# nanoporetech/pomfret

Hardware: AMD Instinct MI355X
Metric: aligned reads/sec (methphase kernel) (higher is better)
Workload: dtype u32/f32

## Files before the change

include/pomfret_amd.h:

```cpp
#ifndef POMFRET_AMD_H
#define POMFRET_AMD_H

#include <stddef.h>
#include <stdint.h>

#ifdef __cplusplus
extern "C" {
#endif

#define PF_ABI_VERSION 1

#define PF_OK               0
#define PF_ERR_ARG         -1
#define PF_ERR_HIP         -2
#define PF_ERR_NOMEM       -3
#define PF_ERR_UNSUPPORTED -4
#define PF_ERR_LIMIT       -5
#define PF_ERR_INTERNAL    -6

typedef struct pf_cfg {
    int32_t k;
    int32_t k_span;
    int32_t cov_for_selection;
    int32_t cov_for_runtime;
// ... 75 lines not shown
#define PF_VAR_D 3

typedef struct pf_known_vars {
    uint32_t n;
    const uint32_t *pos;
    const uint32_t *len;
    const uint8_t  *op;
    const uint8_t  *haptag;
    const uint64_t *char_off;
    const uint8_t  *chars;
} pf_known_vars_t;

typedef struct pf_read_aln_batch {
    uint32_t n_reads;
    const uint32_t *start;
    const uint32_t *end;
    const uint64_t *cigar_off;
    const uint32_t *cigar;
    const uint64_t *seq_off;
    const uint32_t *seq_len;
    const uint8_t  *seq;
    const uint64_t *md_off;
    const char     *md;
} pf_read_aln_batch_t;


typedef struct pf_ctx pf_ctx_t;
typedef struct pf_dbatch pf_dbatch_t;

int  pf_abi_version(void);
int  pf_device_count(void);
const char *pf_strerror(int code);

int  pf_ctx_create(int device, pf_ctx_t **out);
void pf_ctx_destroy(pf_ctx_t *ctx);

int  pf_batch_upload(pf_ctx_t *ctx, const pf_cfg_t *cfg,
                     const pf_window_batch_t *batch, pf_dbatch_t **out);
void pf_batch_free(pf_dbatch_t *db);
uint32_t pf_batch_n_windows(const pf_dbatch_t *db);
uint32_t pf_batch_n_reads(const pf_dbatch_t *db);
uint64_t pf_batch_n_calls(const pf_dbatch_t *db);

int  pf_methphase_run(pf_ctx_t *ctx, pf_dbatch_t *db, pf_window_out_t *out);

int  pf_methphase_launch(pf_ctx_t *ctx, pf_dbatch_t *db);
int  pf_methphase_finish(pf_ctx_t *ctx, pf_dbatch_t *db, pf_window_out_t *out);

int  pf_batch_upload_aln(pf_ctx_t *ctx, const pf_cfg_t *cfg, const pf_load_cfg_t *lcfg,
                         const pf_aln_batch_t *aln, pf_dbatch_t **out);
int  pf_batch_read_recs(const pf_dbatch_t *db, uint32_t *rec_of_read, uint32_t n);
int64_t pf_batch_debug_calls(pf_dbatch_t *db, uint64_t *call_off, uint32_t *pos, uint8_t *cat,
                             uint32_t *first, uint32_t *last, uint64_t cap);

int  pf_batch_debug_recs(pf_dbatch_t *db, uint64_t *sizes, uint16_t *flag, uint8_t *mapq, uint32_t *pos,
                         uint32_t *l_qseq, float *de, uint8_t *hp, uint64_t *cigar_off, uint32_t *cigar,
                         uint64_t *seq_off, uint8_t *seq, uint64_t *mm_off, uint8_t *mm, uint64_t *ml_off,
                         uint8_t *ml);
int  pf_batch_load_counters(pf_dbatch_t *db, uint64_t *out, int n);

int  pf_methphase_windows(int device, const pf_cfg_t *cfg,
                          const pf_window_batch_t *batch, pf_window_out_t *out);

int  pf_last_kernel_times(pf_ctx_t *ctx, const char **names, float *ms, int *n);

int  pf_batch_stats(pf_dbatch_t *db, uint64_t *out, uint64_t n);
int  pf_batch_k3_paths(pf_dbatch_t *db, uint8_t *out, uint64_t n);
int  pf_batch_k12_paths(pf_dbatch_t *db, uint8_t *out, uint64_t n);
int  pf_batch_k12_chunk_items(pf_dbatch_t *db, uint32_t *out);

int  pf_batch_set_mask(pf_dbatch_t *db, const uint32_t *pos, uint64_t n, const uint32_t *win_rng);
int  pf_batch_masked_sites(pf_dbatch_t *db, uint32_t *out, uint64_t n);
int  pf_batch_k3_budget(const pf_dbatch_t *db, uint32_t *out, uint64_t n);

int  pf_batch_heavy(const pf_dbatch_t *db, uint32_t *probs, uint32_t cap);

int  pf_batch_debug_sites(pf_dbatch_t *db, uint32_t w, int dir, uint32_t *real,
                          uint32_t *starts, uint8_t *lens, uint32_t cap);
int64_t pf_batch_debug_methmers(pf_dbatch_t *db, int dir, uint32_t *mmr_n,
                                uint32_t *mmr_start, uint32_t *keys, uint64_t cap);

typedef struct pf_pileup {
    uint32_t n_windows;
    uint64_t n_sites;
    const uint64_t *win_off;
    const uint32_t *pos;
    const uint32_t *cnt;
    float ms_kernels;
} pf_pileup_t;
int  pf_batch_pileup(pf_ctx_t *ctx, pf_dbatch_t *db, const uint8_t *read_hp, uint32_t n_hp, pf_pileup_t **out);
void pf_pileup_free(pf_pileup_t *p);

typedef struct pf_dmr_cfg {
    uint32_t min_cov;
    uint32_t min_delta_pct;
    uint32_t max_gap;
    uint32_t min_sites;
} pf_dmr_cfg_t;

#define PF_DMR_OPEN_LEFT  1u
#define PF_DMR_OPEN_RIGHT 2u
typedef struct pf_dmr_run {
    uint32_t start;
    uint32_t end;
    uint32_t n_sites;
    int32_t  sign;
// ... 609 lines not shown
```

pomfret_amd/_lib.py:

```python
from __future__ import annotations

import ctypes as C
import os
import weakref

import numpy as np

from .abi import (DMR_HMM_SITES, DMR_RUN_DTYPE, REGION_SUM_DTYPE, PfRegions, HmmConfig, PfDmrHmm, PfDmrHmmCfg, AlnBatch, AssignConfig, PfAssign, PfAssignCfg, Config, DmrConfig, KnownVars, LoadConfig, PfAlnBatch, PfCfg, PfDmr, PfDmrCfg,
                  PfKnownVars, PfLoadCfg, PfPerm, PfPileup, PfReadAlnBatch, PfTagcheck, PfWindowBatch, PfWindowOut, ReadAlnBatch,
                  WindowBatch, WindowResult)

_HERE = os.path.dirname(os.path.abspath(__file__))
LIB_PATH = os.path.join(_HERE, "libpomfret_amd.so")
_lib = None


class PomfretError(RuntimeError):
    pass


def lib():
    global _lib
    if _lib is None:
        if not os.path.exists(LIB_PATH):
            raise PomfretError(f"{LIB_PATH} not built: run __graft_entry__.build() or "
                               f"`make -C pomfret_amd/csrc`")
        L = C.CDLL(LIB_PATH)
        L.pf_abi_version.restype = C.c_int
        L.pf_device_count.restype = C.c_int
        L.pf_strerror.restype = C.c_char_p
        L.pf_strerror.argtypes = [C.c_int]
        L.pf_ctx_create.argtypes = [C.c_int, C.POINTER(C.c_void_p)]
        L.pf_ctx_destroy.argtypes = [C.c_void_p]
        L.pf_selftest.argtypes = [C.c_void_p, C.POINTER(C.c_uint64)]
        L.pf_batch_upload.argtypes = [C.c_void_p, C.POINTER(PfCfg), C.POINTER(PfWindowBatch),
                                      C.POINTER(C.c_void_p)]
        L.pf_batch_free.argtypes = [C.c_void_p]
        L.pf_batch_n_windows.argtypes = [C.c_void_p]
        L.pf_batch_n_windows.restype = C.c_uint32
        L.pf_batch_n_reads.argtypes = [C.c_void_p]
        L.pf_batch_n_reads.restype = C.c_uint32
        L.pf_batch_n_calls.argtypes = [C.c_void_p]
        L.pf_batch_n_calls.restype = C.c_uint64
        L.pf_methphase_run.argtypes = [C.c_void_p, C.c_void_p, C.POINTER(PfWindowOut)]
        L.pf_methphase_launch.argtypes = [C.c_void_p, C.c_void_p]
        L.pf_methphase_finish.argtypes = [C.c_void_p, C.c_void_p, C.POINTER(PfWindowOut)]
        L.pf_methphase_windows.argtypes = [C.c_int, C.POINTER(PfCfg), C.POINTER(PfWindowBatch),
                                           C.POINTER(PfWindowOut)]
        L.pf_last_kernel_times.argtypes = [C.c_void_p, C.POINTER(C.c_char_p),
                                           C.POINTER(C.c_float), C.POINTER(C.c_int)]
        L.pf_batch_stats.argtypes = [C.c_void_p, C.c_void_p, C.c_uint64]
        L.pf_batch_heavy.argtypes = [C.c_void_p, C.c_void_p, C.c_uint32]
        L.pf_batch_k3_paths.argtypes = [C.c_void_p, C.c_void_p, C.c_uint64]
        L.pf_batch_k12_paths.argtypes = [C.c_void_p, C.c_void_p, C.c_uint64]
        L.pf_batch_k3_budget.argtypes = [C.c_void_p, C.c_void_p, C.c_uint64]
        L.pf_batch_set_mask.argtypes = [C.c_void_p, C.c_void_p, C.c_uint64, C.c_void_p]
        L.pf_batch_masked_sites.argtypes = [C.c_void_p, C.c_void_p, C.c_uint64]
        L.pf_batch_debug_sites.argtypes = [C.c_void_p, C.c_uint32, C.c_int, C.c_void_p,
                                           C.c_void_p, C.c_void_p, C.c_uint32]
        L.pf_batch_debug_methmers.argtypes = [C.c_void_p, C.c_int, C.c_void_p, C.c_void_p,
                                              C.c_void_p, C.c_uint64]
        L.pf_batch_debug_methmers.restype = C.c_int64
        L.pf_fisher_exact.argtypes = [C.c_int] * 4 + [C.POINTER(C.c_double)] * 3
        L.pf_fisher_exact.restype = C.c_double
        L.pf_batch_upload_aln.argtypes = [C.c_void_p, C.POINTER(PfCfg), C.POINTER(PfLoadCfg),
                                          C.POINTER(PfAlnBatch), C.POINTER(C.c_void_p)]
        L.pf_batch_read_recs.argtypes = [C.c_void_p, C.c_void_p, C.c_uint32]
        L.pf_batch_debug_calls.argtypes = [C.c_void_p] + [C.c_void_p] * 5 + [C.c_uint64]
        L.pf_batch_debug_calls.restype = C.c_int64
        L.pf_batch_load_counters.argtypes = [C.c_void_p, C.c_void_p, C.c_int]
        L.pf_batch_debug_recs.argtypes = [C.c_void_p] * 16
        L.pf_bgzf_inflate.argtypes = [C.c_void_p, C.c_void_p, C.c_uint64, C.c_void_p, C.c_uint64,
                                      C.POINTER(C.c_uint64), C.c_void_p, C.c_uint32, C.POINTER(C.c_float)]
        L.pf_batch_pileup.argtypes = [C.c_void_p, C.c_void_p, C.c_void_p, C.c_uint32,
                                      C.POINTER(C.POINTER(PfPileup))]
        L.pf_pileup_free.argtypes = [C.POINTER(PfPileup)]
        L.pf_write_hapmeth.argtypes = [C.c_char_p, C.c_char_p, C.POINTER(PfPileup), C.c_uint32, C.c_uint32, C.c_int]
        L.pf_dmr_regions.argtypes = [C.c_void_p, C.POINTER(PfPileup), C.c_uint32, C.c_uint32, C.POINTER(PfDmrCfg),
                                     C.c_void_p, C.c_uint32, C.POINTER(C.POINTER(PfDmr))]
        L.pf_dmr_regions_block.argtypes = [C.c_void_p, C.POINTER(PfPileup), C.c_uint32, C.c_uint32, C.POINTER(PfDmrCfg),
                                           C.c_void_p, C.c_uint32, C.c_uint32, C.POINTER(C.POINTER(PfDmr))]
        L.pf_dmr_free.argtypes = [C.POINTER(PfDmr)]
        L.pf_dmr_hmm_regions.argtypes = [C.c_void_p, C.POINTER(PfPileup), C.c_uint32, C.c_uint32, C.POINTER(PfDmrCfg),
                                         C.POINTER(PfDmrHmmCfg), C.c_void_p, C.c_uint32, C.c_uint32, C.c_uint32,
                                         C.POINTER(C.POINTER(PfDmrHmm))]
        L.pf_dmr_hmm_free.argtypes = [C.POINTER(PfDmrHmm)]
        L.pf_dmr_hmm_evidence.argtypes = [C.c_uint32] * 4
        L.pf_dmr_hmm_evidence.restype = C.c_int64
        L.pf_region_sums.argtypes = [C.c_void_p, C.POINTER(PfPileup), C.c_uint32, C.c_uint32, C.POINTER(PfDmrCfg),
                                     C.c_void_p, C.c_void_p, C.c_uint64, C.c_uint32, C.POINTER(C.POINTER(PfRegions))]
        L.pf_regions_free.argtypes = [C.POINTER(PfRegions)]
        L.pf_dmr_acc_new.argtypes = [C.POINTER(PfDmrCfg), C.c_void_p, C.c_uint32]
        L.pf_dmr_acc_new.restype = C.c_void_p
        L.pf_dmr_acc_add.argtypes = [C.c_void_p, C.POINTER(PfDmr)]
        L.pf_dmr_acc_flush.argtypes = [C.c_void_p, C.POINTER(C.POINTER(PfDmr))]
        L.pf_dmr_acc_free.argtypes = [C.c_void_p]
        L.pf_write_dmr.argtypes = [C.c_char_p, C.c_char_p, C.POINTER(PfDmr), C.c_double, C.c_int]
        L.pf_batch_permtest.argtypes = [C.c_void_p, C.c_void_p, C.c_void_p, C.c_uint32, C.c_uint32, C.c_uint32,
                                        C.POINTER(C.POINTER(PfPerm))]
        L.pf_perm_free.argtypes = [C.POINTER(PfPerm)]
        L.pf_write_dmr_perm.argtypes = [C.c_char_p, C.c_char_p, C.POINTER(PfDmr), C.POINTER(PfPerm), C.c_double, C.c_int]
        L.pf_batch_assign.argtypes = [C.c_void_p, C.c_void_p, C.c_void_p, C.c_uint32, C.POINTER(PfAssignCfg),
                                      C.POINTER(C.POINTER(PfAssign))]
        L.pf_assign_free.argtypes = [C.POINTER(PfAssign)]
        L.pf_ilog2_q16.argtypes = [C.c_uint32]
        L.pf_ilog2_q16.restype = C.c_uint32
        L.pf_assign_site_weights.argtypes = [C.c_uint32] * 4 + [C.POINTER(C.c_int32)]
        L.pf_assign_site_weights.restype = None
        L.pf_write_assign.argtypes = [C.c_char_p, C.c_char_p, C.POINTER(PfAssign), C.c_void_p, C.c_void_p, C.c_void_p,
                                      C.c_void_p, C.c_char_p, C.c_int, C.POINTER(C.c_uint64)]
        L.pf_batch_tagcheck.argtypes = [C.c_void_p, C.c_void_p, C.c_void_p, C.c_uint32, C.POINTER(PfAssignCfg),
                                        C.POINTER(C.POINTER(PfTagcheck))]
        L.pf_tagcheck_free.argtypes = [C.POINTER(PfTagcheck)]
        L.pf_tagcheck_site_weights.argtypes = [C.c_uint32] * 5 + [C.POINTER(C.c_int32), C.POINTER(C.c_uint8)]
        L.pf_tagcheck_site_weights.restype = None
        L.pf_write_tagcheck.argtypes = [C.c_char_p, C.c_char_p, C.POINTER(PfTagcheck), C.c_void_p, C.c_void_p, C.c_void_p,
                                        C.c_void_p, C.c_char_p, C.c_int, C.POINTER(C.c_uint64)]
        L.pf_write_tagcheck_regions.argtypes = [C.c_char_p, C.c_char_p, C.POINTER(PfTagcheck), C.c_void_p, C.c_void_p,
                                                C.c_int, C.POINTER(C.c_uint64)]
        if hasattr(L, "pf_haptag_reads"):
            L.pf_haptag_reads.argtypes = [C.c_void_p, C.POINTER(PfKnownVars),
                                          C.POINTER(PfReadAlnBatch), C.c_void_p]
# ... 385 lines not shown

    def debug_recs(self) -> dict:
        sz = np.zeros(5, np.uint64)
        _check(lib().pf_batch_debug_recs(self.handle, sz.ctypes.data, *([None] * 14)), "pf_batch_debug_recs")
        n, nc, ns, nm, nl = (int(x) for x in sz)
        d = dict(flag=np.zeros(n, np.uint16), mapq=np.zeros(n, np.uint8), pos=np.zeros(n, np.uint32),
                 l_qseq=np.zeros(n, np.uint32), de=np.zeros(n, np.float32), hp=np.zeros(n, np.uint8),
                 cigar_off=np.zeros(n + 1, np.uint64), cigar=np.zeros(max(nc, 1), np.uint32),
                 seq_off=np.zeros(n + 1, np.uint64), seq=np.zeros(max(ns, 1), np.uint8),
                 mm_off=np.zeros(n + 1, np.uint64), mm=np.zeros(max(nm, 1), np.uint8),
                 ml_off=np.zeros(n + 1, np.uint64), ml=np.zeros(max(nl, 1), np.uint8))
        keys = ["flag", "mapq", "pos", "l_qseq", "de", "hp", "cigar_off", "cigar", "seq_off", "seq", "mm_off", "mm",
                "ml_off", "ml"]
        _check(lib().pf_batch_debug_recs(self.handle, sz.ctypes.data, *[d[k].ctypes.data for k in keys]),
               "pf_batch_debug_recs")
        d["cigar"], d["seq"], d["mm"], d["ml"] = d["cigar"][:nc], d["seq"][:ns], d["mm"][:nm], d["ml"][:nl]
        return d

    @property
    def n_reads(self) -> int:
        return int(lib().pf_batch_n_reads(self.handle))

    def read_recs(self) -> np.ndarray:
        R = self.n_reads
        out = np.zeros(max(R, 1), np.uint32)
        rc = lib().pf_batch_read_recs(self.handle, out.ctypes.data, out.size)
        if rc != 0 and self.record_level:
            self.debug_calls(cap=0, probe=True)
            R = self.n_reads
            rc = lib().pf_batch_read_recs(self.handle, out.ctypes.data, out.size)
        _check(rc, "pf_batch_read_recs")
        return out[:R]

    def debug_calls(self, cap: int = None, probe: bool = False):
        if cap is None:
            if self.record_level and not lib().pf_batch_n_calls(self.handle):
                self.debug_calls(cap=0, probe=True)
            cap = int(lib().pf_batch_n_calls(self.handle))
        R = self.n_reads
        off = np.zeros(R + 1, np.uint64)
        pos = np.zeros(max(cap, 1), np.uint32)
        cat = np.zeros(max(cap, 1), np.uint8)
        first = np.zeros(max(R, 1), np.uint32)
        last = np.zeros(max(R, 1), np.uint32)
        n = lib().pf_batch_debug_calls(self.handle, off.ctypes.data, pos.ctypes.data, cat.ctypes.data,
                                       first.ctypes.data, last.ctypes.data, cap)
        if probe:
            return None
        if n < 0:
            _check(int(n), "pf_batch_debug_calls")
        R = self.n_reads
        return off[:R + 1], pos[:n], cat[:n], first[:R], last[:R]

    def load_counters(self) -> dict:
        out = np.zeros(8, np.uint64)
        _check(lib().pf_batch_load_counters(self.handle, out.ctypes.data, 8), "pf_batch_load_counters")
        return dict(seq_path=int(out[0]), unsorted=int(out[1]), implicit=int(out[2]), bad_mm=int(out[3]),
                    dup_chunks=int(out[4]), multi_cm=int(out[5]))

    def free(self):
        if self.handle:
            lib().pf_batch_free(self.handle)
            self.handle = None

    def __del__(self):
        try:
            self.free()
        except Exception:
            pass

    def run(self, out: WindowResult = None) -> WindowResult:
        fresh = out is None
        if fresh:
            out = WindowResult.alloc(self.n_windows, self.n_reads)
        o = out.to_c()
        _check(lib().pf_methphase_run(self.ctx.handle, self.handle, C.byref(o)), "pf_methphase_run")
        if fresh:
            out.read_hp = out.read_hp[:self.n_reads]
        return out

    def pileup(self, read_hp=None) -> dict:
        hp_ptr, n_hp = None, 0
        if read_hp is not None:
            hp = np.zeros(np.size(read_hp) + 1, np.uint8)
            hp[:-1] = np.asarray(read_hp, np.uint8).ravel()
            hp_ptr, n_hp = hp.ctypes.data, hp.size - 1
        p = C.POINTER(PfPileup)()
        _check(lib().pf_batch_pileup(self.ctx.handle, self.handle, hp_ptr, n_hp, C.byref(p)), "pf_batch_pileup")
        try:
            r = p.contents
            W, n = int(r.n_windows), int(r.n_sites)
            win_off = np.ctypeslib.as_array(r.win_off, (W + 1,)).copy()
            pos = np.ctypeslib.as_array(r.pos, (n,)).copy() if n else np.zeros(0, np.uint32)
            cnt = np.ctypeslib.as_array(r.cnt, (n * 6,)).copy() if n else np.zeros(0, np.uint32)
            return dict(win_off=win_off, pos=pos, cnt=cnt.reshape(n, 3, 2), ms=float(r.ms_kernels))
        finally:
            lib().pf_pileup_free(p)

    def permtest(self, n_perm: int, seed: int = 1, read_hp=None) -> dict:
        hp_ptr, n_hp = None, 0
        if read_hp is not None:
            hp = np.zeros(np.size(read_hp) + 1, np.uint8)
            hp[:-1] = np.asarray(read_hp, np.uint8).ravel()
            hp_ptr, n_hp = hp.ctypes.data, hp.size - 1
        if not 0 <= int(n_perm) <= 0xFFFFFFFF or not 0 <= int(seed) <= 0xFFFFFFFF:
            raise PomfretError("pf_batch_permtest: n_perm and seed are 32-bit unsigned")
# ... 161 lines not shown
```

pomfret_amd/csrc/pf_api.hip:

```cpp
#include <hip/hip_runtime.h>
#include <mutex>
#include <stdint.h>
#include <stdio.h>
#include <stdlib.h>
#include <string.h>
#include <algorithm>
#include <thread>
#include <vector>
#include "pf_device.h"
#include "pf_load.h"
#include "pf_host.h"
#include "../../include/pomfret_amd.h"

__global__ void pf_k12_sites_methmers(pf_dev_batch d);
__global__ void pf_k2_methmers(pf_dev_batch d);
__global__ void pf_k12_chunks(pf_dev_batch d);
__global__ void pf_k3_greedy(pf_dev_batch d);
__global__ void pf_k3_wave(pf_dev_batch d);
__global__ void pf_k3_fallback(pf_dev_batch d);
__global__ void pf_k3_heavy(pf_dev_batch d);
__global__ void pf_k3_kdict(pf_dev_batch d);
__global__ void pf_k0_load(pf_load_dev d);
__global__ void pf_k0_multi(pf_load_dev d);
__global__ void pf_k0_scan(pf_load_dev d);
// ... 1604 lines not shown
        }
    }
    *n = tot;
    return PF_OK;
}

extern "C" int64_t pf_batch_debug_calls(pf_dbatch_t *b, uint64_t *call_off, uint32_t *pos, uint8_t *cat,
                                        uint32_t *first, uint32_t *last, uint64_t cap) {
    if (!b || !call_off || !pos || !cat || !first || !last) return PF_ERR_ARG;
    const int rc = run_debug(b, 0);
    if (rc) return rc;
    if (b->N > cap) return PF_ERR_ARG;
    if (b->R == 0) { call_off[0] = 0; return 0; }
    const uint32_t *dpos = b->d.call_pos;
    const uint8_t *dcat = b->d.call_cat;
    if (b->has_aln) {
        std::vector<uint64_t> beg(b->R), end(b->R);
        HIPCHK(hipMemcpy(beg.data(), b->d.read_call_off, 8ull * b->R, hipMemcpyDeviceToHost));
        HIPCHK(hipMemcpy(end.data(), b->d.read_call_end, 8ull * b->R, hipMemcpyDeviceToHost));
        call_off[0] = 0;
        for (uint32_t r = 0; r < b->R; r++) call_off[r + 1] = call_off[r] + (end[r] - beg[r]);
        if (call_off[b->R] != b->N) return PF_ERR_INTERNAL;
        if (b->dbg_cap < b->N || !b->dbg_off) {
            if (b->dbg_off) { free_arena(b, b->dbg_off); free_arena(b, b->dbg_pos); free_arena(b, b->dbg_cat); }
            b->dbg_off = nullptr; b->dbg_pos = nullptr; b->dbg_cat = nullptr; b->dbg_cap = 0;
            int ra = dev_alloc(b, &b->dbg_off, (size_t)b->ld.n_recs + 1);
            if (!ra) ra = dev_alloc(b, &b->dbg_pos, (size_t)b->N);
            if (!ra) ra = dev_alloc(b, &b->dbg_cat, (size_t)b->N);
            if (ra) return ra;
            b->dbg_cap = b->N;
        }
        hipStream_t st = b->ctx->stream;
        HIPCHK(hipMemcpyAsync(b->dbg_off, call_off, 8ull * (b->R + 1), hipMemcpyHostToDevice, st));
        hipLaunchKernelGGL(pf_k0_gather_calls, dim3(std::min<uint32_t>((b->R + 3) / 4, 4096)), dim3(256), 0, st,
                           b->d.read_call_off, b->dbg_off, b->R, b->d.call_pos, b->d.call_cat, b->dbg_pos, b->dbg_cat);
        HIPCHK(hipGetLastError());
        HIPCHK(hipStreamSynchronize(st));
        dpos = b->dbg_pos;
        dcat = b->dbg_cat;
    } else {
        HIPCHK(hipMemcpy(call_off, b->d.read_call_off, 8ull * (b->R + 1), hipMemcpyDeviceToHost));
    }
    if (b->N) {
        HIPCHK(hipMemcpy(pos, dpos, 4ull * b->N, hipMemcpyDeviceToHost));
        HIPCHK(hipMemcpy(cat, dcat, b->N, hipMemcpyDeviceToHost));
    }
    if (b->R) {
        HIPCHK(hipMemcpy(first, b->d.read_first, 4ull * b->R, hipMemcpyDeviceToHost));
        HIPCHK(hipMemcpy(last, b->d.read_last, 4ull * b->R, hipMemcpyDeviceToHost));
    }
    return (int64_t)b->N;
}

extern "C" int pf_batch_set_hp(pf_dbatch_t *b, const uint8_t *hp, uint32_t n) {
    if (!b || !b->has_aln || n != b->ld.n_recs || (n && !hp)) return PF_ERR_ARG;
    if (!n) return PF_OK;
    HIPCHK(hipSetDevice(b->ctx->device));
    HIPCHK(hipStreamSynchronize(b->ctx->stream));
    HIPCHK(hipMemcpy(const_cast<uint8_t *>(b->ld.hp), hp, n, hipMemcpyHostToDevice));
    return PF_OK;
}

extern "C" int pf_batch_set_mask(pf_dbatch_t *b, const uint32_t *pos, uint64_t n, const uint32_t *win_rng) {
    if (!b || (n && !pos)) return PF_ERR_ARG;
    for (uint64_t i = 0; i < n; i++) {
        if (i && pos[i] <= pos[i - 1]) return PF_ERR_ARG;
        if (pos[i] >= (1u << 29)) return PF_ERR_LIMIT;
    }
    if (n && win_rng)
        for (uint32_t w = 0; w < b->W; w++)
            if (win_rng[2 * w] > win_rng[2 * w + 1] || win_rng[2 * w + 1] > n) return PF_ERR_ARG;
    HIPCHK(hipSetDevice(b->ctx->device));
    HIPCHK(hipStreamSynchronize(b->ctx->stream));
    uint32_t *np = nullptr, *nr = nullptr;
    int rc = PF_OK;
    if (n) {
        rc = dev_put(b, &np, pos, (size_t)n);
        if (!rc && win_rng && b->W) rc = dev_put(b, &nr, win_rng, 2ull * b->W);
        if (rc) {
            if (np) free_arena(b, np);
            if (nr) free_arena(b, nr);
            return rc;
        }
    }
    pf_dev_batch &d = b->d;
    if (d.mask_pos) free_arena(b, const_cast<uint32_t *>(d.mask_pos));
    if (d.win_mask_rng) free_arena(b, const_cast<uint32_t *>(d.win_mask_rng));
    d.mask_pos = np;
    d.win_mask_rng = nr;
    d.mask_n = (uint32_t)n;
    return PF_OK;
}

extern "C" int pf_batch_masked_sites(pf_dbatch_t *b, uint32_t *out, uint64_t n) {
    if (!b || !out || n < b->W) return PF_ERR_ARG;
    HIPCHK(hipSetDevice(b->ctx->device));
    HIPCHK(hipStreamSynchronize(b->ctx->stream));
    if (b->W) HIPCHK(hipMemcpy(out, b->d.win_masked, 4ull * b->W, hipMemcpyDeviceToHost));
    return PF_OK;
}

extern "C" int pf_batch_debug_recs(pf_dbatch_t *b, uint64_t *sizes, uint16_t *flag, uint8_t *mapq, uint32_t *pos,
                                   uint32_t *l_qseq, float *de, uint8_t *hp, uint64_t *cigar_off, uint32_t *cigar,
                                   uint64_t *seq_off, uint8_t *seq, uint64_t *mm_off, uint8_t *mm, uint64_t *ml_off,
                                   uint8_t *ml) {
    if (!b || !sizes || !b->has_aln) return PF_ERR_ARG;
// ... 46 lines not shown
```

pomfret_amd/csrc/pf_load.hip:

```cpp
#include <hip/hip_runtime.h>
#include <stdint.h>
#include "pf_device.h"
#include "pf_load.h"

#define DEV static __device__ __forceinline__
#define NT_C 2u
#ifndef PF_K0_SEQ_REREAD
#define PF_K0_SEQ_REREAD 0
#endif

#ifdef PF_K0_PROFILE
DEV unsigned long long k0_now() {
    unsigned long long t;
    __builtin_amdgcn_sched_barrier(0);
    asm volatile("s_memtime %0\n\ts_waitcnt lgkmcnt(0)" : "=s"(t) :: "memory");
    __builtin_amdgcn_sched_barrier(0);
    return t;
}
#define K0_STAMP(i) do { const unsigned long long t_ = k0_now(); \
    if (d->ctr && lane == 0) atomicAdd(&d->ctr[8 + (i)], t_ - k0_t); k0_t = t_; } while (0)
#define K0_T0 unsigned long long k0_t = k0_now()
#else
#define K0_STAMP(i) do { } while (0)
#define K0_T0 do { } while (0)
#endif
#define NT_G 4u
#ifndef PF_K0_NOINL
#define PF_K0_NOINL 0
#endif
#if PF_K0_NOINL & 1
#define DEV_HBM static __device__ __attribute__((noinline))
#else
#define DEV_HBM DEV
#endif
#if PF_K0_NOINL & 2
#define DEV_COLD static __device__ __attribute__((noinline))
#else
#define DEV_COLD DEV
#endif
#ifndef PF_K0_PLACE
#define PF_K0_PLACE 1
#endif
#ifndef PF_K0_WALK2
#define PF_K0_WALK2 1
#endif
#ifndef PF_K0_FUSEC
#define PF_K0_FUSEC 1
#endif
#ifndef PF_K0_PADFIX
#define PF_K0_PADFIX 1
#endif
#ifndef PF_K0_NBRARE
#define PF_K0_NBRARE 1
#endif
#ifndef PF_K0_RANKDPP
#define PF_K0_RANKDPP 1
#endif
#ifndef PF_K0_HDRFAST
#define PF_K0_HDRFAST 1
#endif
#ifndef PF_K0_EMITDPP
#define PF_K0_EMITDPP 1
#endif
#ifndef PF_K0_DIAG1
#define PF_K0_DIAG1 0
#endif
#if PF_K0_DIAG1
#define K0_DIAG1(d) ((d)->diag == 1u)
#else
#define K0_DIAG1(d) false
#endif
#ifndef PF_K0_WPE
#define PF_K0_WPE 8
#endif

DEV uint32_t uni(uint32_t x) { return (uint32_t)__builtin_amdgcn_readfirstlane((int)x); }
DEV uint64_t lanemask_lt(uint32_t lane) { return lane ? (~0ull >> (64 - lane)) : 0ull; }
DEV uint32_t popc(uint64_t m) { return (uint32_t)__popcll(m); }
DEV uint32_t below_cnt(uint64_t b) {
    return __builtin_amdgcn_mbcnt_hi((uint32_t)(b >> 32), __builtin_amdgcn_mbcnt_lo((uint32_t)b, 0u));
}
DEV uint32_t rdl(uint32_t x, uint32_t l) { return (uint32_t)__builtin_amdgcn_readlane((int)x, (int)l); }

#define K0_CONST __attribute__((address_space(4)))
typedef const K0_CONST pf_load_dev *K0Args;
typedef const K0_CONST pf_k0_hdr *K0HdrP;
DEV K0Args k0_args() { return (K0Args)__builtin_amdgcn_kernarg_segment_ptr(); }
template <typename P>
DEV P k0_late(P p) {
    asm volatile("" : "+s"(p));
    return p;
}

DEV void wsync() {
    __builtin_amdgcn_fence(__ATOMIC_RELEASE, "workgroup");
    __builtin_amdgcn_wave_barrier();
    __builtin_amdgcn_fence(__ATOMIC_ACQUIRE, "workgroup");
}

DEV uint32_t dpp_shr_add(uint32_t x, const int ctrl) {
    uint32_t y;
    switch (ctrl) {
    case 1: y = (uint32_t)__builtin_amdgcn_update_dpp(0, (int)x, 0x111, 0xF, 0xF, true); break;
    case 2: y = (uint32_t)__builtin_amdgcn_update_dpp(0, (int)x, 0x112, 0xF, 0xF, true); break;
    case 4: y = (uint32_t)__builtin_amdgcn_update_dpp(0, (int)x, 0x114, 0xF, 0xF, true); break;
    case 8: y = (uint32_t)__builtin_amdgcn_update_dpp(0, (int)x, 0x118, 0xF, 0xF, true); break;
    case 15: y = (uint32_t)__builtin_amdgcn_update_dpp(0, (int)x, 0x142, 0xA, 0xF, false); break;
    default: y = (uint32_t)__builtin_amdgcn_update_dpp(0, (int)x, 0x143, 0xC, 0xF, false); break;
    }
    return x + y;
}
DEV uint32_t wscan(uint32_t x, uint32_t) {
    x = dpp_shr_add(x, 1);
    x = dpp_shr_add(x, 2);
    x = dpp_shr_add(x, 4);
// ... 1 lines not shown
    x = dpp_shr_add(x, 15);
    x = dpp_shr_add(x, 31);
    return x;
}
DEV uint64_t wscan64(uint64_t x, uint32_t lane) {
#pragma unroll
    for (int o = 1; o < 64; o <<= 1) {
        const uint64_t y = __shfl_up(x, o, 64);
        if (lane >= (uint32_t)o) x += y;
    }
    return x;
}
DEV uint64_t rdl64(uint64_t x, uint32_t l) {
    return ((uint64_t)rdl((uint32_t)(x >> 32), l) << 32) | rdl((uint32_t)x, l);
}

DEV uint32_t nib(const uint8_t *s, uint32_t i) { return (s[i >> 1] >> ((~i & 1u) << 2)) & 0xFu; }
DEV uint32_t nibw(uint64_t w, uint32_t i) { return (uint32_t)(w >> (8u * (i >> 1) + ((i & 1u) ? 0u : 4u))) & 0xFu; }
DEV uint32_t match16(uint64_t w, uint32_t tb, uint32_t nv) {
    uint32_t m = 0;
#pragma unroll
    for (uint32_t i = 0; i < 16; i++) m |= (nibw(w, i) == tb && i < nv) ? (1u << i) : 0u;
    return m;
}
DEV uint32_t select_bit(uint32_t m, uint32_t k) {
    for (uint32_t i = 0; i < k; i++) m &= m - 1;
    return (uint32_t)__builtin_ctz(m);
}
DEV bool is_digit(uint32_t c) { return c >= '0' && c <= '9'; }
DEV bool is_alpha(uint32_t c) { return (c >= 'a' && c <= 'z') || (c >= 'A' && c <= 'Z'); }

template <bool LE>
DEV uint32_t lb64(const uint32_t *a, uint32_t n, uint32_t v) {
    uint32_t lo = 0;
    while (n > 0) {
        const uint32_t h = n >> 1;
        const uint32_t x = a[lo + h];
        if (LE ? x <= v : x < v) { lo += h + 1; n -= h + 1; } else n = h;
    }
    return lo;
}

struct K0Merge {
    uint32_t eP[PF_K0_EC], eV[PF_K0_EC];
    uint32_t iP[PF_K0_EC], iV[PF_K0_EC];
    uint32_t mV[2 * PF_K0_EC];
    uint8_t eC[PF_K0_EC];
    uint8_t mC[2 * PF_K0_EC];
};
struct K0Seq {
    uint16_t sb[8 * 64];
    uint8_t sc[8 * 64];
};
struct K0W {
    uint32_t T[PF_K0_TCAP];
    uint32_t opE[64], opOff[64], opA[64];
    uint8_t opT[64];
    union {
        K0Seq s;
        K0Merge mg;
    } u;
};

struct K0Out {
    uint32_t n, first, last;
    uint32_t sorted, lim;
    uint32_t *pos;
    uint8_t *cat;
};

struct K0Tgt { uint32_t nd, nc, mi, th, te; uint64_t ml; };
#define PF_K0_MAXT 8
#define PF_K0_TW 7
struct K0Tgts { K0Tgt t0; uint32_t n, over; uint32_t *xt; };
DEV void k0_tgt_put(uint32_t *xt, uint32_t e, const K0Tgt &t, uint32_t lane) {
    if (lane == 0) {
        uint32_t *q = xt + PF_K0_TW * (e - 1);
        q[0] = t.nd; q[1] = t.nc; q[2] = t.mi; q[3] = t.th; q[4] = t.te; q[5] = (uint32_t)t.ml;
        q[6] = (uint32_t)(t.ml >> 32);
    }
}
DEV K0Tgt k0_tgt_get(const K0Tgts &T, uint32_t e) {
    if (e == 0) return T.t0;
    const uint32_t *q = T.xt + PF_K0_TW * (e - 1);
    K0Tgt t;
    t.nd = q[0]; t.nc = q[1]; t.mi = q[2]; t.th = q[3]; t.te = q[4];
    t.ml = ((uint64_t)q[6] << 32) | q[5];
    return t;
}

DEV uint32_t bytes_eq(uint32_t w, uint32_t c) {
    const uint32_t t = w ^ (c * 0x01010101u);
    return ~(((t & 0x7F7F7F7Fu) + 0x7F7F7F7Fu) | t) & 0x80808080u;
}
DEV uint32_t bytes_in(int32_t b, uint32_t lo, uint32_t hi) {
    const int32_t s = min(max((int32_t)lo - b, 0), 4), e = min(max((int32_t)hi - b, 0), 4);
    const uint32_t ml = s >= 4 ? 0u : 0x80808080u << (8 * s);
    const uint32_t mh = e <= 0 ? 0u : 0x80808080u >> (8 * (4 - e));
    return ml & mh;
}
DEV uint32_t wsum_small(uint32_t c) {
    return popc(__ballot(c & 1u)) + 2u * popc(__ballot(c & 2u)) + 4u * popc(__ballot(c & 4u));
}
DEV uint64_t nondigit_bytes(uint64_t y) {
    const uint64_t hi = (y & 0xF0F0F0F0F0F0F0F0ull) ^ 0x3030303030303030ull;
    const uint64_t hz = ~(((hi & 0x7F7F7F7F7F7F7F7Full) + 0x7F7F7F7F7F7F7F7Full) | hi) & 0x8080808080808080ull;
    const uint64_t ge10 = ((y & 0x0F0F0F0F0F0F0F0Full) + 0x7676767676767676ull) & 0x8080808080808080ull;
    return (~hz & 0x8080808080808080ull) | ge10;
}
DEV uint32_t swar_dec(uint64_t y, uint32_t n) {
    uint64_t z = (y & ((1ull << (8 * n)) - 1)) << (8 * (8 - n));
    z = ((z & 0x0F0F0F0F0F0F0F0Full) * 2561u) >> 8;
    z = ((z & 0x00FF00FF00FF00FFull) * 6553601u) >> 16;
    return (uint32_t)(((z & 0x0000FFFF0000FFFFull) * 42949672960001ull) >> 32);
}
// ... 338 lines not shown
DEV uint32_t u16_at(uint4 q, uint32_t e) {
    const uint32_t d = e < 2 ? q.x : e < 4 ? q.y : e < 6 ? q.z : q.w;
    return (e & 1u) ? d >> 16 : d & 0xFFFFu;
}
DEV uint64_t valid_nibbles(uint32_t nv) { return nv >= 16 ? 0x1111111111111111ull : ((1ull << (4 * nv)) - 1) & 0x1111111111111111ull; }

template <typename TP>
DEV uint32_t k0_seq_pass(K0Args d, K0W &L, const uint8_t *seq, uint32_t len, bool rev, const K0Tgt &t,
                         TP TB, uint32_t lane, bool &implicit, uint32_t &tb_off) {
    constexpr uint32_t ROWS = 8, RW = 128, BW = ROWS * RW;
    const uint64_t pat = (rev ? (uint64_t)NT_G : (uint64_t)NT_C) * 0x1111111111111111ull;
    const uint4 *sq4 = reinterpret_cast<const uint4 *>(seq);
    const uint32_t nwords = (len + 15) / 16;
    const uint32_t nblk = (nwords + BW - 1) / BW;
    const uint32_t nd = t.nd;
    auto slot = [&](uint32_t j) { return rev ? nd - 1 - j : j; };
    uint32_t carry = 0, ti = 0, nout = 0;
    bool imp = false;
    tb_off = 0;
    for (uint32_t bb = 0; bb < nblk && ti < nd; bb++) {
        const uint32_t b = rev ? nblk - 1 - bb : bb;
        uint4 v[ROWS];
        const uint32_t w0 = b * BW + 2 * lane;
        const int32_t left = (int32_t)(nwords - w0);
        const uint4 *rowp = sq4 + (w0 >> 1);
#pragma unroll
        for (uint32_t i = 0; i < ROWS; i++)
            v[i] = (int32_t)(i * RW) < left ? rowp[i * (RW / 2)] : make_uint4(0, 0, 0, 0);
        uint32_t pref[ROWS];
        uint32_t run = 0;
        auto count = [&](uint32_t i, uint32_t &c0) {
            const uint32_t w = b * BW + i * RW + 2 * lane;
            const uint64_t xs[2] = {((uint64_t)v[i].y << 32) | v[i].x, ((uint64_t)v[i].w << 32) | v[i].z};
            uint32_t c[2];
#pragma unroll
            for (uint32_t h = 0; h < 2; h++) {
#if PF_K0_PADFIX
                (void)w;
                c[h] = (uint32_t)__popcll(zero_nibbles_hi(xs[h] ^ pat));
#else
                c[h] = 0;
                if (w + h < nwords) {
                    if ((w + h) * 16 + 16 > len)
                        c[h] = (uint32_t)__popcll(zero_nibbles(nibswap(xs[h]) ^ pat) & valid_nibbles(len - (w + h) * 16));
                    else c[h] = (uint32_t)__popcll(zero_nibbles_hi(xs[h] ^ pat));
                }
#endif
            }
            c0 = c[0];
            return c[0] + c[1];
        };
#pragma unroll
        for (uint32_t i = 0; i < ROWS; i += 2) {
            uint32_t c0a, c0b;
            const uint32_t ca = count(i, c0a), cb = count(i + 1, c0b);
            L.u.s.sc[i * 64 + lane] = (uint8_t)c0a;
            L.u.s.sc[(i + 1) * 64 + lane] = (uint8_t)c0b;
            const uint32_t inc = wscan(ca | (cb << 16), lane);
            const uint32_t tot = rdl(inc, 63);
            pref[i] = run;
            const uint32_t ba = run + (inc & 0xFFFFu) - ca;
            L.u.s.sb[i * 64 + lane] = (uint16_t)ba;
            run += tot & 0xFFFFu;
            pref[i + 1] = run;
            const uint32_t bb2 = run + (inc >> 16) - cb;
            L.u.s.sb[(i + 1) * 64 + lane] = (uint16_t)bb2;
            run += tot >> 16;
#if PF_K0_PLACE
            if ((lane & 7u) == 0) {
                uint16_t *gb = reinterpret_cast<uint16_t *>(L.opA);
                gb[i * 8 + (lane >> 3)] = (uint16_t)ba;
                gb[(i + 1) * 8 + (lane >> 3)] = (uint16_t)bb2;
            }
#endif
        }
        const uint32_t btot = run;
        uint32_t tend = ti;
#if PF_K0_PLACE
        {
            const uint32_t lim = carry + btot;
            uint32_t lo = ti, n = nd - ti;
            while (n > 64) {
                const uint32_t sd = (n + 63) / 64, off = lane * sd;
                const bool in = off < n && (TB[slot(min(lo + off, nd - 1))] & 0xFFFFFFu) < lim;
                const uint32_t c = popc(__ballot(in));
                if (c == 0) { n = 0; break; }
                const uint32_t nlo = lo + (c - 1) * sd + 1;
                n = min(c * sd, n) - (c - 1) * sd - 1;
                lo = nlo;
            }
            const bool in = lane < n && (TB[slot(min(lo + lane, nd - 1))] & 0xFFFFFFu) < lim;
            tend = uni(lo + popc(__ballot(in)));
        }
#else
        {
            uint32_t n = nd - ti;
            while (n > 0) {
                const uint32_t h = n >> 1;
                if ((TB[slot(tend + h)] & 0xFFFFFFu) < carry + btot) { tend += h + 1; n -= h + 1; } else n = h;
            }
            tend = uni(tend);
        }
#endif
        wsync();
        for (uint32_t j0 = ti; j0 < (d->diag == 5u ? ti : tend); j0 += 64) {
            const uint32_t j = j0 + lane;
// ... 476 lines not shown
                const uint32_t p = key >> 2;
                const bool in = k < nT && p <= a_end;
                const uint64_t bi = __ballot(in);
                if (!bi) break;
                bool keep = false;
                uint32_t v = 0;
                if (in) {
#if PF_K0_WALK2
                    auto lt8 = [&](uint4 x, uint4 y) {
                        return (x.x < p ? 1u : 0u) + (x.y < p ? 1u : 0u) + (x.z < p ? 1u : 0u) + (x.w < p ? 1u : 0u) +
                               (y.x < p ? 1u : 0u) + (y.y < p ? 1u : 0u) + (y.z < p ? 1u : 0u) + (y.w < p ? 1u : 0u);
                    };
                    const uint4 *gl = reinterpret_cast<const uint4 *>(L.u.mg.eP);
                    const uint32_t g = lt8(gl[0], gl[1]);
                    const uint4 *ge = reinterpret_cast<const uint4 *>(L.opE + 8 * g);
                    const uint32_t oi = 8 * g + lt8(ge[0], ge[1]);
#else
                    const uint32_t oi = lb64<false>(L.opE, nv, p);
#endif
                    keep = L.opT[oi] == 0;
                    v = i_ref + p + cgoffset + L.opOff[oi];
                }
                k0_emit_lanes<MODE>(d, o, keep, v, key & 3u, false, lane, L.u.mg.mV, L.u.mg.mC);
                tc += popc(bi);
                if (popc(bi) < 64) break;
            }
        } else {
            for (uint32_t c0 = a_cur & ~3u; c0 <= a_end && (c0 < a_end || tc < nT); c0 += PF_K0_CB)
                k0_chunk_implicit<MODE>(d, L, nv, c0, a_cur, a_end, i_ref, cgoffset, rev, TB, nT, tc, seq, len,
                                        lane, o);
        }
        wsync();
        a_cur = a_end;
        off_cur = off_end;
        j += 64;
    }
    for (; j < ncig; j += 64) {
        const uint32_t g = j + lane;
        const uint32_t c = cn;
        next_tile();
        racc += k0_refc(c);
        if (trunc) continue;
        const uint32_t op = c & 15u;
        const uint64_t stop = __ballot(op == 3u || op == 4u);
        const uint64_t bad = __ballot(op > 4u && g < ncig);
        const uint32_t fs = stop ? (uint32_t)__ffsll((long long)stop) - 1 : 64u;
        const uint32_t fb = bad ? (uint32_t)__ffsll((long long)bad) - 1 : 64u;
        if (fb < fs) return false;
        trunc = fs < 64;
    }
    return true;
}

DEV K0HdrP k0_rec(K0Args d, uint32_t slot) { return (K0HdrP)(d->hdr + slot); }

template <typename TP>
DEV bool k0_merge_targets(K0Args d, K0W &L, const K0Tgts &T, uint32_t N, bool rev, TP TB,
                          const uint32_t *gw, const uint8_t *mmg, uint32_t mis, const uint8_t *ml, uint32_t mln,
                          uint32_t lane, uint32_t &nd_out, bool &past, bool &ovf) {
    nd_out = 0;
    ovf = false;
    unsigned long long t0 = 0;
    if (lane == 0) t0 = atomicAdd(d->stage_ctr, 2ull * N);
    const uint64_t cb = d->stage_off[d->n_recs] + (((uint64_t)uni((uint32_t)(t0 >> 32)) << 32) | uni((uint32_t)t0));
    if (cb + 2ull * N > d->stage_cap) {
        if (lane == 0) atomicOr(d->status, PF_ST_STAGE_OVF);
        ovf = true;
        return false;
    }
    uint32_t *tmp = d->stage_pos + cb, *mrg = tmp + N;
    k0_dw_table(L.u.mg.mV, lane);
    wsync();
    bool pst = false;
    for (uint32_t e = 0, oe = 0; e < T.n; e++) {
        const K0Tgt te = k0_tgt_get(T, e);
        uint32_t *TBe = tmp + oe;
        if (!k0_mm_ranks(gw, mmg, mis, te, rev, TBe, L.u.mg.mV, lane)) return false;
        wsync();
        for (uint32_t j = lane; j < te.nd; j += 64) {
            const uint32_t q = mln ? (uint32_t)ml[te.ml + (uint64_t)j * te.nc + te.mi] : 255u;
            const uint32_t sj = rev ? te.nd - 1 - j : j;
            const uint32_t rk = TBe[sj];
            pst |= rk >= (1u << 24);
            TBe[sj] = (rk & 0xFFFFFFu) | (q << 24);
        }
        wsync();
        oe += te.nd;
    }
    past = __ballot(pst) != 0;
    if (past) return true;
    for (uint32_t e = 0, oe = 0; e < T.n; e++) {
        const uint32_t ne = k0_tgt_get(T, e).nd;
        for (uint32_t j = lane; j < ne; j += 64) {
            const uint32_t v = tmp[oe + (rev ? ne - 1 - j : j)], rk = v & 0xFFFFFFu;
            uint32_t pos = j;
            for (uint32_t f = 0, of = 0; f < T.n; f++) {
                const uint32_t nf = k0_tgt_get(T, f).nd;
                if (f != e) {
                    uint32_t lo = 0, hi = nf;
                    while (lo < hi) {
                        const uint32_t mid = (lo + hi) >> 1;
                        const uint32_t x = tmp[of + (rev ? nf - 1 - mid : mid)] & 0xFFFFFFu;
                        if (f < e ? x <= rk : x < rk) lo = mid + 1;
                        else hi = mid;
                    }
                    pos += lo;
// ... 95 lines not shown
    }
    K0_STAMP(0);
    d = k0_late(d);
    h = k0_late(h);
    if (d->diag == 2u) { if (lane == 0) d->rec_n[h->rec] = PF_NONE; return; }
    const uint8_t *seq = d->seq + h->seq_off;
    const uint32_t len = h->l_qseq;
    uint32_t tb_off = 0;
    if (okmm && t.nd && !past) nT = k0_seq_pass(d, L, seq, len, rev, t, TB, lane, implicit, tb_off);
    TB = TB + uni(tb_off);
    K0_STAMP(1);
    d = k0_late(d);
    h = k0_late(h);
    const uint32_t r = h->rec;
    if (d->diag == 3u || d->diag == 5u) { if (lane == 0) d->rec_n[r] = PF_NONE; return; }
    const uint32_t ncig = h->ncig;
    const uint32_t *cig = d->cigar + h->cig_off;
    if (!okmm && d->ctr && lane == 0) atomicAdd(&d->ctr[PF_K0C_BADMM], 1ull);
    nT = uni(nT);

    if (ncig == 0 || nT == 0) {
        if (lane == 0) d->rec_n[r] = PF_NONE;
        return;
    }
    uint64_t cb = h->stage_off;
    if (implicit || nT > h->stage_len) {
        const uint64_t need = (uint64_t)nT + (uint64_t)(len + 1) / 2;
        unsigned long long t = 0;
        if (lane == 0) t = atomicAdd(d->stage_ctr, (unsigned long long)need);
        cb = d->stage_off[d->n_recs] + (((uint64_t)uni((uint32_t)(t >> 32)) << 32) | uni((uint32_t)t));
        if (cb + need > d->stage_cap) {
            if (lane == 0) { atomicOr(d->status, PF_ST_STAGE_OVF); d->rec_n[r] = PF_NONE; }
            return;
        }
    }
    K0Out o;
    o.n = 0; o.first = 0; o.last = 0; o.sorted = 1; o.lim = 0;
    o.pos = d->stage_pos + cb;
    o.cat = d->stage_cat + cb;
    if (implicit && d->ctr && lane == 0) atomicAdd(&d->ctr[PF_K0C_IMPLICIT], 1ull);

    const uint32_t qs = h->pos;
    const bool stale = (cig[0] & 15u) == 4u && (TB[nT - 1] >> 2) <= (cig[0] >> 4);
    bool fatal = false, walked = false;
    uint32_t racc = 0;
    if (stale || d->force_seq) {
        if (d->ctr && lane == 0) atomicAdd(&d->ctr[PF_K0C_SEQPATH], 1ull);
        K0Out s = o;
        bool f = false;
        if (lane == 0) k0_walk_seq<1>(cig, ncig, qs, rev, TB, nT, implicit ? seq : nullptr, len, s, f);
        k0_bcast(o, s);
        fatal = uni(f ? 1u : 0u) != 0;
    } else {
        fatal = !k0_walk<1>(d, L, cig, ncig, qs, rev, TB, nT, seq, len, implicit, lane, o, racc);
        walked = true;
    }
    K0_STAMP(2);
    if (fatal) {
        if (lane == 0) { atomicOr(d->status, PF_ST_FATAL_CIGAR); d->rec_n[r] = PF_NONE; }
        return;
    }
    if (o.lim && lane == 0) atomicOr(d->status, PF_ST_POS_LIMIT);
    if (!o.sorted && o.n > 1) {
        if (d->ctr && lane == 0) atomicAdd(&d->ctr[PF_K0C_UNSORTED], 1ull);
        __builtin_amdgcn_fence(__ATOMIC_RELEASE, "agent");
        if (lane == 0) {
            for (uint32_t i = 1; i < o.n; i++) {
                const uint32_t v = o.pos[i];
                const uint8_t cc = o.cat[i];
                uint32_t k = i;
                while (k > 0 && (o.pos[k - 1] > v || (o.pos[k - 1] == v && o.cat[k - 1] > cc))) {
                    o.pos[k] = o.pos[k - 1];
                    o.cat[k] = o.cat[k - 1];
                    k--;
                }
                o.pos[k] = v;
                o.cat[k] = cc;
            }
        }
    }
    uint32_t rlen = racc;
    if (!walked)
        for (uint32_t c = lane; c < ncig; c += 64) rlen += k0_refc(cig[c]);
    rlen = rdl(wscan(rlen, lane), 63);
    if (lane < 8) {
        const uint32_t v = lane == 0 ? qs : lane == 1 ? qs + rlen : lane == 2 ? o.first : lane == 3 ? o.last
                         : lane == 4 ? (uint32_t)cb : lane == 5 ? (uint32_t)(cb >> 32) : 0u;
        d->rec_out[8ull * r + lane] = v;
    }
    if (lane == 63) {
        d->rec_n[r] = o.n;
        const uint32_t w = h->rec_win;
        atomicAdd(&d->win_kept[w], 1u);
        atomicAdd(&d->win_calls[w], o.n);
    }
    K0_STAMP(3);
}

template <bool MULTI>
DEV_HBM void k0_record_hbm(K0Args d, K0W &L, K0HdrP h, uint32_t lane, const K0Tgts &T, bool okm) {
    k0_record<MULTI>(d, L, h, lane, d->scr + h->scr_off, h->scr_len, T, okm);
}

template <bool MULTI>
DEV void k0_one(K0Args d, K0W &L, uint32_t slot, uint32_t lane) {
    const K0HdrP h = k0_rec(d, slot);
    const uint32_t fm = h->flag_mapq, flag = fm & 0xFFFFu, len = h->l_qseq;
// ... 173 lines not shown
```

Measured before the change: 60.63 million.

## Walk CIGAR in 128-op tiles per wave and skip empty prefix rows

Adds a CIGAR walker that processes two ops per lane (128 per wave tile), using a two-level LDS search (segment and group end arrays) to map target positions to CIGAR ops. This is used for non-implicit records. It also skips prefix-count rows beyond the record's word count, and adds a debug spans API. The aim is to halve tile iterations and ballots for long CIGARs, at the cost of union-overlaid LDS layout and extra search logic.

```diff
diff --git a/include/pomfret_amd.h b/include/pomfret_amd.h
--- a/include/pomfret_amd.h
+++ b/include/pomfret_amd.h
@@ -151,6 +151,7 @@
 int  pf_batch_read_recs(const pf_dbatch_t *db, uint32_t *rec_of_read, uint32_t n);
 int64_t pf_batch_debug_calls(pf_dbatch_t *db, uint64_t *call_off, uint32_t *pos, uint8_t *cat,
                              uint32_t *first, uint32_t *last, uint64_t cap);
+int  pf_batch_debug_spans(pf_dbatch_t *db, uint32_t *start, uint32_t *end, uint32_t n);
 
 int  pf_batch_debug_recs(pf_dbatch_t *db, uint64_t *sizes, uint16_t *flag, uint8_t *mapq, uint32_t *pos,
                          uint32_t *l_qseq, float *de, uint8_t *hp, uint64_t *cigar_off, uint32_t *cigar,
diff --git a/pomfret_amd/_lib.py b/pomfret_amd/_lib.py
--- a/pomfret_amd/_lib.py
+++ b/pomfret_amd/_lib.py
@@ -68,6 +68,7 @@
         L.pf_batch_read_recs.argtypes = [C.c_void_p, C.c_void_p, C.c_uint32]
         L.pf_batch_debug_calls.argtypes = [C.c_void_p] + [C.c_void_p] * 5 + [C.c_uint64]
         L.pf_batch_debug_calls.restype = C.c_int64
+        L.pf_batch_debug_spans.argtypes = [C.c_void_p, C.c_void_p, C.c_void_p, C.c_uint32]
         L.pf_batch_load_counters.argtypes = [C.c_void_p, C.c_void_p, C.c_int]
         L.pf_batch_debug_recs.argtypes = [C.c_void_p] * 16
         L.pf_bgzf_inflate.argtypes = [C.c_void_p, C.c_void_p, C.c_uint64, C.c_void_p, C.c_uint64,
@@ -559,6 +560,13 @@
         R = self.n_reads
         return off[:R + 1], pos[:n], cat[:n], first[:R], last[:R]
 
+    def debug_spans(self):
+        n = max(self.n_reads, 1)
+        start, end = np.zeros(n, np.uint32), np.zeros(n, np.uint32)
+        _check(lib().pf_batch_debug_spans(self.handle, start.ctypes.data, end.ctypes.data, n), "pf_batch_debug_spans")
+        R = self.n_reads
+        return start[:R], end[:R]
+
     def load_counters(self) -> dict:
         out = np.zeros(8, np.uint64)
         _check(lib().pf_batch_load_counters(self.handle, out.ctypes.data, 8), "pf_batch_load_counters")
diff --git a/pomfret_amd/csrc/pf_api.hip b/pomfret_amd/csrc/pf_api.hip
--- a/pomfret_amd/csrc/pf_api.hip
+++ b/pomfret_amd/csrc/pf_api.hip
@@ -1680,6 +1680,18 @@
     return (int64_t)b->N;
 }
 
+extern "C" int pf_batch_debug_spans(pf_dbatch_t *b, uint32_t *start, uint32_t *end, uint32_t n) {
+    if (!b || !start || !end) return PF_ERR_ARG;
+    const int rc = run_debug(b, 0);
+    if (rc) return rc;
+    if (b->R > n) return PF_ERR_ARG;
+    if (b->R) {
+        HIPCHK(hipMemcpy(start, b->d.read_start, 4ull * b->R, hipMemcpyDeviceToHost));
+        HIPCHK(hipMemcpy(end, b->d.read_end, 4ull * b->R, hipMemcpyDeviceToHost));
+    }
+    return PF_OK;
+}
+
 extern "C" int pf_batch_set_hp(pf_dbatch_t *b, const uint8_t *hp, uint32_t n) {
     if (!b || !b->has_aln || n != b->ld.n_recs || (n && !hp)) return PF_ERR_ARG;
     if (!n) return PF_OK;
diff --git a/pomfret_amd/csrc/pf_load.hip b/pomfret_amd/csrc/pf_load.hip
--- a/pomfret_amd/csrc/pf_load.hip
+++ b/pomfret_amd/csrc/pf_load.hip
@@ -61,6 +61,12 @@
 #endif
 #ifndef PF_K0_EMITDPP
 #define PF_K0_EMITDPP 1
+#endif
+#ifndef PF_K0_ROWSKIP
+#define PF_K0_ROWSKIP 1
+#endif
+#ifndef PF_K0_TILE128
+#define PF_K0_TILE128 1
 #endif
 #ifndef PF_K0_DIAG1
 #define PF_K0_DIAG1 0
@@ -168,15 +174,28 @@
     uint16_t sb[8 * 64];
     uint8_t sc[8 * 64];
 };
+struct K0Wide {
+    uint32_t E[128], Off[128];
+    uint32_t gE[16], sE[4];
+    uint8_t T[128];
+    uint32_t mV[64];
+    uint8_t mC[64];
+};
 struct K0W {
     uint32_t T[PF_K0_TCAP];
-    uint32_t opE[64], opOff[64], opA[64];
-    uint8_t opT[64];
     union {
-        K0Seq s;
-        K0Merge mg;
-    } u;
+        struct {
+            uint32_t opE[64], opOff[64], opA[64];
+            uint8_t opT[64];
+            union {
+                K0Seq s;
+                K0Merge mg;
+            } u;
+        };
+        K0Wide w;
+    };
 };
+static_assert(sizeof(K0W) == 5120, "K0W: 5 KB per wave, 20,480 B per block");
 
 struct K0Out {
     uint32_t n, first, last;
@@ -621,6 +640,13 @@
         };
 #pragma unroll
         for (uint32_t i = 0; i < ROWS; i += 2) {
+#if PF_K0_ROWSKIP
+            if (i * RW >= nwords - b * BW) {
+                pref[i] = run;
+                pref[i + 1] = run;
+                continue;
+            }
+#endif
             uint32_t c0a, c0b;
             const uint32_t ca = count(i, c0a), cb = count(i + 1, c0b);
             L.u.s.sc[i * 64 + lane] = (uint8_t)c0a;
@@ -1203,6 +1229,103 @@
     return true;
 }
 
+#if PF_K0_TILE128
+template <int MODE, typename TP>
+DEV bool k0_walk128(K0Args d, K0W &L, const uint32_t *cig, uint32_t ncig, uint32_t qs, bool rev, TP TB,
+                    uint32_t nT, uint32_t lane, K0Out &o, uint32_t &racc) {
+    K0Wide &W = L.w;
+    const uint32_t cgoffset = rev ? 0xFFFFFFFFu : 0u;
+    uint32_t a_cur = 0, off_cur = 0, j = 0, tc = 0, i_ref = qs;
+    if ((cig[0] & 15u) == 4u) {
+        const uint32_t sclip = cig[0] >> 4;
+        tc = k0_tlb(TB, nT, sclip + 1);
+        if (tc > 0 && (TB[tc - 1] >> 2) == sclip) k0_emit_one<MODE>(o, qs + cgoffset, TB[tc - 1] & 3u, false);
+        i_ref = qs - sclip;
+        a_cur = sclip;
+        j = 1;
+    }
+    bool trunc = false;
+    auto ld_tile = [&](uint32_t t) {
+        const uint32_t g = t + 2 * lane;
+        return make_uint2(g < ncig ? cig[g] : 4u, g + 1 < ncig ? cig[g + 1] : 4u);
+    };
+    uint2 cn = ld_tile(j);
+    auto next_tile = [&]() { cn = j + 128 < ncig ? ld_tile(j + 128) : make_uint2(4u, 4u); };
+    auto first_of = [](uint64_t even, uint64_t odd) {
+        const uint32_t fe = even ? 2u * ((uint32_t)__ffsll((long long)even) - 1) : 128u;
+        const uint32_t fo = odd ? 2u * ((uint32_t)__ffsll((long long)odd) - 1) + 1u : 128u;
+        return min(fe, fo);
+    };
+    auto tile_stop = [&](uint32_t op0, uint32_t op1, uint32_t &fs) {
+        fs = first_of(__ballot(op0 == 3u || op0 == 4u), __ballot(op1 == 3u || op1 == 4u));
+        return first_of(__ballot(op0 > 4u), __ballot(op1 > 4u)) >= fs;
+    };
+    while (j < ncig && !trunc && tc < nT) {
+        const uint2 c = cn;
+        next_tile();
+        racc += k0_refc(c.x) + k0_refc(c.y);
+        const uint32_t op0 = c.x & 15u, op1 = c.y & 15u, ln0 = c.x >> 4, ln1 = c.y >> 4;
+        uint32_t nv;
+        if (!tile_stop(op0, op1, nv)) return false;
+        trunc = nv < 128;
+        const bool v0 = 2 * lane < nv, v1 = 2 * lane + 1 < nv;
+        const uint32_t rl0 = v0 && op0 <= 1u ? ln0 : 0u, rl1 = v1 && op1 <= 1u ? ln1 : 0u;
+        const uint32_t dl0 = !v0 ? 0u : op0 == 2u ? ln0 : op0 == 1u ? 0u - ln0 : 0u;
+        const uint32_t dl1 = !v1 ? 0u : op1 == 2u ? ln1 : op1 == 1u ? 0u - ln1 : 0u;
+        const uint32_t rs = rl0 + rl1, ds = dl0 + dl1;
+        const uint32_t rin = wscan(rs, lane), din = wscan(ds, lane);
+        const uint32_t a0 = a_cur + rin - rs, off0 = off_cur + din - ds;
+        const uint32_t oe1 = v1 ? a0 + rs : 0xFFFFFFFFu;
+        reinterpret_cast<uint2 *>(W.E)[lane] = make_uint2(v0 ? a0 + rl0 : 0xFFFFFFFFu, oe1);
+        reinterpret_cast<uint2 *>(W.Off)[lane] = make_uint2(off0, off0 + dl0);
+        reinterpret_cast<uint16_t *>(W.T)[lane] = (uint16_t)(op0 | (op1 << 8));
+        if ((lane & 3u) == 3u) W.gE[lane >> 2] = oe1;
+        if ((lane & 15u) == 15u) W.sE[lane >> 4] = oe1;
+        const uint32_t a_end = a_cur + rdl(rin, 63);
+        const uint32_t off_end = off_cur + rdl(din, 63);
+        wsync();
+        for (;;) {
+            const uint32_t k = tc + lane;
+            const uint32_t key = k < nT ? TB[k] : 0xFFFFFFFFu;
+            const uint32_t p = key >> 2;
+            const bool in = k < nT && p <= a_end;
+            const uint64_t bi = __ballot(in);
+            if (!bi) break;
+            bool keep = false;
+            uint32_t v = 0;
+            if (in) {
+                auto lt4 = [&](uint4 x) {
+                    return (x.x < p ? 1u : 0u) + (x.y < p ? 1u : 0u) + (x.z < p ? 1u : 0u) + (x.w < p ? 1u : 0u);
+                };
+                const uint32_t s = lt4(*reinterpret_cast<const uint4 *>(W.sE));
+                const uint32_t g = 4 * s + lt4(reinterpret_cast<const uint4 *>(W.gE)[s]);
+                const uint4 *ge = reinterpret_cast<const uint4 *>(W.E + 8 * g);
+                const uint32_t oi = 8 * g + lt4(ge[0]) + lt4(ge[1]);
+                keep = W.T[oi] == 0;
+                v = i_ref + p + cgoffset + W.Off[oi];
+            }
+            k0_emit_lanes<MODE>(d, o, keep, v, key & 3u, false, lane, W.mV, W.mC);
+            tc += popc(bi);
+            if (popc(bi) < 64) break;
+        }
+        wsync();
+        a_cur = a_end;
+        off_cur = off_end;
+        j += 128;
+    }
+    for (; j < ncig; j += 128) {
+        const uint2 c = cn;
+        next_tile();
+        racc += k0_refc(c.x) + k0_refc(c.y);
+        if (trunc) continue;
+        uint32_t fs;
+        if (!tile_stop(c.x & 15u, c.y & 15u, fs)) return false;
+        trunc = fs < 128;
+    }
+    return true;
+}
+#endif
+
 DEV K0HdrP k0_rec(K0Args d, uint32_t slot) { return (K0HdrP)(d->hdr + slot); }
 
 template <typename TP>
@@ -1404,7 +1527,12 @@
         k0_bcast(o, s);
         fatal = uni(f ? 1u : 0u) != 0;
     } else {
+#if PF_K0_TILE128
+        if (!implicit) fatal = !k0_walk128<1>(d, L, cig, ncig, qs, rev, TB, nT, lane, o, racc);
+        else fatal = !k0_walk<1>(d, L, cig, ncig, qs, rev, TB, nT, seq, len, true, lane, o, racc);
+#else
         fatal = !k0_walk<1>(d, L, cig, ncig, qs, rev, TB, nT, seq, len, implicit, lane, o, racc);
+#endif
         walked = true;
     }
     K0_STAMP(2);
```

After: 61.85 million (median of 6 runs). 1.02x the previous value.
